# 0215Arthur/Pytorch_News_Recommender

Hardware: AMD Instinct MI355X
Metric: users/sec (train step) NRMS MIND-small hist=50 cand=5 (higher is better)
Workload: dtype f16 (MFMA inputs and saved activations; fp32 accumulate, softmax, loss, master weights and Adam)

## Files before the change

include/nrms_hip.h:

```cpp
#ifndef NRMS_HIP_H
#define NRMS_HIP_H

#include <stddef.h>
#include <stdint.h>

#ifdef __cplusplus
extern "C" {
#endif

#define NRMS_OK            0
#define NRMS_EINVAL       -1
#define NRMS_ELAUNCH      -2
#define NRMS_EWORKSPACE   -3

#define NRMS_PRECISION_FP32   0
#define NRMS_PRECISION_BF16X3 1
#define NRMS_PRECISION_BF16   2
#define NRMS_FP16_KP 320
#define NRMS_FP16_DP 320
#define NRMS_FP16_QP 224
#define NRMS_PRECISION_FP16   3

#define NRMS_FLAG_PAD_ROW_ZERO 1
#define NRMS_FLAG_DEFER_WQKV 2
// ... 46 lines not shown
    float* qkv;
    float* attn;
    float* ctx;
    float* t;
    float* w;
    void*  scratch;
} nrms_encoder_acts;

size_t nrms_encoder_fwd_scratch_bytes(const nrms_encoder_desc* desc);
size_t nrms_encoder_fused_qkv_bytes(const nrms_encoder_desc* desc);
int nrms_encoder_fwd(const nrms_encoder_desc* desc, const nrms_encoder_weights* w,
                     const int64_t* ids, const float* x, const uint8_t* mask ,
                     const nrms_encoder_acts* acts, float* out, void* stream);

size_t nrms_encoder_bwd_workspace_bytes(const nrms_encoder_desc* desc);
int nrms_encoder_bwd(const nrms_encoder_desc* desc, const nrms_encoder_weights* w,
                     const int64_t* ids, const float* x, const uint8_t* mask,
                     const nrms_encoder_acts* acts, const float* dout,
                     const nrms_encoder_grads* grads, float* dx,
                     void* workspace, size_t workspace_bytes, void* stream);
int nrms_encoder_bwd_wqkv(const nrms_encoder_desc* desc, const int64_t* ids, const float* x,
                          const nrms_encoder_acts* acts, const nrms_encoder_grads* grads,
                          void* workspace, size_t workspace_bytes, void* stream);

int nrms_sanitize_ids(const int64_t* src, int64_t* dst, int64_t n, int32_t vocab, int32_t* n_bad, void* stream);
int nrms_sanitize_ids_i32(const int32_t* src, int64_t* dst, int64_t n, int32_t vocab, int32_t* n_bad, void* stream);

int nrms_title_dedup(const int64_t* ids, int64_t n_titles, int32_t seq_len, int32_t* table, int64_t table_size,
                     int32_t* inverse, int32_t* rep_rows, int32_t* n_unique, void* stream);

// ... 118 lines not shown
```

pytorch_news_recommender_amd/_lib.py:

```python
from __future__ import annotations

import ctypes as C
import os

PKG = os.path.dirname(os.path.abspath(__file__))
LIB_PATH = os.environ.get("NRMS_HIP_LIB") or os.path.join(PKG, "libnrms_hip.so")

NRMS_FLAG_PAD_ROW_ZERO = 1
NRMS_FLAG_DEFER_WQKV = 2
NRMS_FLAG_FWD_SCRATCH_KEPT = 4
NRMS_FLAG_FUSED_SEQ64 = 8
NRMS_PRECISION_FP32 = 0
NRMS_PRECISION_BF16X3 = 1
NRMS_PRECISION_BF16 = 2
NRMS_PRECISION_FP16 = 3
NRMS_DROPOUT_FIELDS16 = 0x100
NRMS_FP16_KP, NRMS_FP16_DP, NRMS_FP16_QP = 320, 320, 224
PRECISIONS = {"fp32": 0, "bf16x3": 1, "bf16": 2, "fp16": 3}


class NrmsError(RuntimeError):
    pass


# ... 26 lines not shown


NRMS_SEGPOOL_ROWS_UNIQUE = 1


class NewsFeatures(C.Structure):
    _fields_ = [("n", C.c_int64), ("d_text", C.c_int32), ("d_cat", C.c_int32), ("n_cat", C.c_int32), ("n_sub", C.c_int32),
                ("p_drop", C.c_float), ("seed", C.c_uint64), ("title_vec", C.c_void_p), ("abst_vec", C.c_void_p),
                ("cat_table", C.c_void_p), ("sub_table", C.c_void_p), ("categ", C.c_void_p), ("subcateg", C.c_void_p)]


SIGNATURES = {
    "nrms_encoder_fwd": (C.c_int, [C.POINTER(EncoderDesc), C.POINTER(EncoderWeights), C.c_void_p, C.c_void_p,
                                   C.c_void_p, C.POINTER(EncoderActs), C.c_void_p, C.c_void_p]),
    "nrms_encoder_bwd_workspace_bytes": (C.c_size_t, [C.POINTER(EncoderDesc)]),
    "nrms_encoder_fwd_scratch_bytes": (C.c_size_t, [C.POINTER(EncoderDesc)]),
    "nrms_encoder_fused_qkv_bytes": (C.c_size_t, [C.POINTER(EncoderDesc)]),
    "nrms_encoder_bwd": (C.c_int, [C.POINTER(EncoderDesc), C.POINTER(EncoderWeights), C.c_void_p, C.c_void_p,
                                   C.c_void_p, C.POINTER(EncoderActs), C.c_void_p, C.POINTER(EncoderGrads), C.c_void_p,
                                   C.c_void_p, C.c_size_t, C.c_void_p]),
    "nrms_encoder_bwd_wqkv": (C.c_int, [C.POINTER(EncoderDesc), C.c_void_p, C.c_void_p, C.POINTER(EncoderActs),
                                        C.POINTER(EncoderGrads), C.c_void_p, C.c_size_t, C.c_void_p]),
    "nrms_sanitize_ids": (C.c_int, [C.c_void_p, C.c_void_p, C.c_int64, C.c_int32, C.c_void_p, C.c_void_p]),
    "nrms_sanitize_ids_i32": (C.c_int, [C.c_void_p, C.c_void_p, C.c_int64, C.c_int32, C.c_void_p, C.c_void_p]),
    "nrms_title_dedup": (C.c_int, [C.c_void_p, C.c_int64, C.c_int32, C.c_void_p, C.c_int64, C.c_void_p, C.c_void_p,
                                   C.c_void_p, C.c_void_p]),
    "nrms_click_score_indexed": (C.c_int, [C.c_int32, C.c_int32, C.c_int32, C.c_void_p, C.c_int64, C.c_void_p, C.c_void_p,
                                           C.c_void_p, C.c_void_p, C.c_void_p]),
    "nrms_click_score_fwd": (C.c_int, [C.c_int32, C.c_int32, C.c_int32, C.c_void_p, C.c_void_p, C.c_void_p,
                                       C.c_void_p, C.c_void_p]),
# ... 81 lines not shown
```

pytorch_news_recommender_amd/csrc/capi.hip:

```cpp
#include <stdarg.h>

#include <algorithm>

#include <mutex>
#include <vector>

#include "gemm.h"

namespace nrms {

int launch_attention(bool bwd, int n_seq, int S, int d, int h, const float* qkv, float* ctx, const Dropout& drop,
                     const float* dctx, float* dqkv, const uint8_t* mask, const int64_t* ids, const float* bias_hm,
                     const int* pos, float* padsum, float* dbias, hipStream_t stream, const Dropout* pdrop = nullptr,
                     bool split = false);
size_t attention_padsum_floats();
int launch_addattn_fwd(int n_seq, int S, int d, int q, const float* ctx, const float* w_add, const float* b_add,
                       const float* q_vec, float* T, float* wout, float* out, const uint8_t* mask, int npass,
                       void* wplanes, hipStream_t stream);
int addattn_bwd_rows_waves(int n_seq);
int launch_addattn_bwd_rows(int n_seq, int S, int d, int q, const float* ctx, const float* dout, const float* w,
                            const float* T, float* ds, float* dq_partial, float* dq, const uint8_t* mask,
                            hipStream_t stream);

int launch_attention_wide(bool bwd, int n_seq, int S, int d, int h, const float* qkv, float* ctx, const Dropout& pdrop,
// ... 536 lines not shown
    if (desc->precision == NRMS_PRECISION_FP16) return fwd16_scratch(desc).total;
    return fwd_scratch(desc).total;
}

extern "C" size_t nrms_encoder_fused_qkv_bytes(const nrms_encoder_desc* desc) {
    if (desc == nullptr || !(desc->flags & NRMS_FLAG_FUSED_SEQ64) || validate_desc(desc, "encoder_fused_qkv_bytes")) return 0;
    return user64_qkv_bytes(desc->n_seq, desc->n_heads);
}

extern "C" size_t nrms_encoder_bwd_workspace_bytes(const nrms_encoder_desc* desc) {
    if (validate_desc(desc, "encoder_bwd_workspace_bytes")) return 0;
    if (desc->precision == NRMS_PRECISION_FP16) return bwd16_layout(desc).total;
    return bwd_layout(desc).total;
}

namespace nrms {
struct SideEntry { int device; hipStream_t caller; SideSet* set; };
static std::mutex g_side_mu;
static std::vector<SideEntry> g_side_sets;

SideSet* side_streams_for(hipStream_t caller) {
    if (getenv("NRMS_NO_SIDE_STREAMS") != nullptr) return nullptr;
    int dev = 0;
    if (hipGetDevice(&dev) != hipSuccess) return nullptr;
    std::lock_guard<std::mutex> lk(g_side_mu);
    for (const SideEntry& e : g_side_sets)
        if (e.device == dev && e.caller == caller) return e.set;
    if (g_side_sets.size() >= 32) return nullptr;
    SideSet* ss = new SideSet();
    bool ok = true;
// ... 344 lines not shown
```

pytorch_news_recommender_amd/csrc/fused16_bwd.h:

```cpp
#pragma once
#include "fused16.h"

namespace nrms {

constexpr int B16_RED_QKV = 3 * 10 * 32;
constexpr int B16_RED = B16_RED_QKV + 2 * F16_QP;
constexpr int B16_DQ = 96 * 10;

struct Bwd16Args {
    int n_seq, S, d, h, dk, q;
    int n_groups;
    const _Float16* x16;
    const int* pos;
    const int* n_rows;
    const int64_t* ids;
    const int* order;
    const int* order_cnt;
    int n_cls;
    const _Float16* btiles;
    const float* bqkv32;
    const _Float16* qv16;
    const _Float16* ctx16;
    const _Float16* t16;
    const float* w;
    const _Float16* dout16;
    _Float16* dz16;
    _Float16* dctx16;
    _Float16* dqkv16;
    float* red;
    Dropout drop;
    int v1;
    int dbg;
};

__device__ __forceinline__ f32x16 transpose32(const f32x16& x, const h8 (&idf)[2]) {
    f32x16 z = mfma32h(acc_frag(x, 0), idf[0], zero16());
    return mfma32h(acc_frag(x, 1), idf[1], z);
}

__device__ __forceinline__ float regsum(const f32x16& x) {
    float s0 = 0.f, s1 = 0.f, s2 = 0.f, s3 = 0.f;
#pragma unroll
    for (int g = 0; g < 4; ++g) { s0 += x[4 * g]; s1 += x[4 * g + 1]; s2 += x[4 * g + 2]; s3 += x[4 * g + 3]; }
    return (s0 + s1) + (s2 + s3);
}

__device__ __forceinline__ f32x16 transpose_frags(const h8& x0, const h8& x1, const h8 (&idf)[2]) {
    f32x16 z = mfma32h(x0, idf[0], zero16());
// ... 13 lines not shown
    const _Float16* xtiles;
    int lda, n_slabs;
    float* c;
    int ldc, d;
    const float* sc;
};


size_t bwd16_fused_lds(bool two_blocks);
int launch_bwd16_pool(const Bwd16Args& a, int n_wg, bool two_blocks, hipStream_t stream);
int launch_dx16(const Dx16Args& g, bool out16, hipStream_t stream);
int launch_dout16(long n_seq, int d, int h, int dk, float fixed_scale, float* sc, const float* dout, _Float16* dout16, hipStream_t stream);
int launch_tn16(int geom, const _Float16* A, int lda, int N, const _Float16* B, int ldb, int K, int M, const int* m_dev,
                float* partial, int splits, const int* nmap, const int* kmap, const float* nscale, int ldw, float* dW,
                hipStream_t stream, const char* name, float* dbias = nullptr, const int* blk_list = nullptr, const int* blk_cnt = nullptr,
                int blk_stride = 0);

}
```

pytorch_news_recommender_amd/csrc/fused16_bwd.hip:

```cpp
#include <stdlib.h>

#include "fused16_bwd.h"

namespace nrms {

template <int SB>
__global__ __launch_bounds__(F16_THREADS, SB == 1 ? 8 / F16_WAVES : 1) void fused_bwd16_pool_kernel(Bwd16Args a) {
    extern __shared__ __attribute__((aligned(16))) char smem[];
    float* red = reinterpret_cast<float*>(smem + 3 * F16_SLOT);
    float* stg_t = red + B16_RED;
    float* stg_h = stg_t + F16_WAVES * SB * 2 * F16_QT * 32;
    const int tid = threadIdx.x, lane = tid & 63;
    const int wave = __builtin_amdgcn_readfirstlane(tid >> 6);
    const int l32 = lane & 31, hh = lane >> 5;
    const int S = a.S;
    constexpr int DP = F16_DP, QP = F16_QP;

    for (int i = tid; i < B16_RED; i += F16_THREADS) red[i] = 0.f;

    h8 idf[2], sel[2];
#pragma unroll
    for (int s = 0; s < 2; ++s)
#pragma unroll
        for (int j = 0; j < 8; ++j) {
// ... 84 lines not shown
        for (int b = 0; b < SB; ++b) {
            const float ds = wgt[b] * (dw[b] - aw);
            const _Float16* tsrc = a.t16 + frag_off((long)seq * SB + b, QP / 16, 0, l32, hh);
#pragma unroll
            for (int s = 0; s < 14; ++s) zf[b][s] = *reinterpret_cast<const h8*>(tsrc + 512 * s);
#pragma unroll
            for (int t = 0; t < F16_QT; ++t) {
                f32x16 accz = zero16(), accu = zero16();
#pragma unroll
                for (int s2 = 0; s2 < 2; ++s2) {
                    const int s = 2 * t + s2;
                    const h8 qf = *reinterpret_cast<const h8*>(a.qv16 + 16 * s + 8 * hh);
                    h8 dz, u;
#pragma unroll
                    for (int j = 0; j < 8; ++j) {
                        const float tv = (float)zf[b][s][j];
                        dz[j] = (_Float16)(ds * (float)qf[j] * (1.0f - tv * tv));
                        u[j] = (_Float16)(ds * tv);
                    }
                    zf[b][s] = dz;
                    if (valid && !F16_DBG(a.dbg, 4)) *reinterpret_cast<h8*>(a.dz16 + frag_off((long)seq * SB + b, QP / 16, s, l32, hh)) = dz;
                    accz = mfma32h(dz, sel[s2], accz);
                    accu = mfma32h(u, sel[s2], accu);
                }
                float cz = valid ? regsum(accz) : 0.f, cu = valid ? regsum(accu) : 0.f;
                cz += __shfl_xor(cz, 32, 64);
                cu += __shfl_xor(cu, 32, 64);
                if (hh == 0) {
                    float* row = stg_t + ((wave * SB + b) * 2 * F16_QT + 2 * t) * 32 + l32;
                    row[0] = cz;
                    row[32] = cu;
                }
            }
            zf[b][14] = h8{0, 0, 0, 0, 0, 0, 0, 0};
            zf[b][15] = h8{0, 0, 0, 0, 0, 0, 0, 0};
        }
        ring.store(0);
        ring.load(1);
        ring.store(1);
        const bool any_closed = __syncthreads_or((!live && valid) ? 1 : 0) != 0;
        for (int i = tid; i < 2 * F16_QT * 32; i += F16_THREADS) {
            float sum = 0.f;
#pragma unroll
            for (int w = 0; w < F16_WAVES; ++w)
#pragma unroll
                for (int b = 0; b < SB; ++b) sum += stg_t[((w * SB + b) * 2 * F16_QT) * 32 + i];
            const int r = i >> 5, c = i & 31;
            red[B16_RED_QKV + (r & 1) * QP + 32 * (r >> 1) + c] += sum;
        }

        int n = 0;
#pragma unroll 1
        for (int head = 0; head < a.h; ++head) {
            ring.load(n + 2);
            const h8 d0 = *reinterpret_cast<const h8*>(a.dout16 + (long)seq * DP + head * 32 + 8 * hh);
            const h8 d1 = *reinterpret_cast<const h8*>(a.dout16 + (long)seq * DP + head * 32 + 16 + 8 * hh);
            float closed = 0.f;
#pragma unroll
            for (int b = 0; b < SB; ++b) {
                f32x16 dct = zero16();
                if (!F16_DBG(a.dbg, 8)) tile_mma<true>(dct, ring, n, zf[b]);
#pragma unroll
                for (int r = 0; r < 8; ++r) {
                    dct[r] += wgt[b] * (float)d0[r];
                    dct[8 + r] += wgt[b] * (float)d1[r];
                }
                if (a.drop.thresh != 0u) {
#pragma unroll
                    for (int c = 0; c < 2; ++c) {
                        const uint64_t e0 = (uint64_t)(tok0 + 32 * b + l32) * (uint64_t)DP + (uint64_t)(head * 32 + 16 * c + 8 * hh);
                        float sc[8];
// ... 551 lines not shown
    static constexpr int STAGE = A_BYTES + B_BYTES;
    static constexpr int A_IT = (T16_MC * AW / 8 + T16_THREADS - 1) / T16_THREADS;
    static constexpr int B_IT = (T16_MC * BW / 8 + T16_THREADS - 1) / T16_THREADS;
};
typedef Tn16Geom<4, 5, 2, 5> Tn16Qkv;
typedef Tn16Geom<2, 7, 4, 5> Tn16Add;

struct Tn16Args {
    int M;
    const int* m_dev;
    const _Float16* A; int lda, N;
    const _Float16* B; int ldb, K;
    float* partial;
    int splits, n_blk, k_blk;
    const int* blk_list; const int* blk_cnt; int blk_stride;
};

typedef short s16x4 __attribute__((ext_vector_type(4)));
typedef short s16x8 __attribute__((ext_vector_type(8)));

__device__ __forceinline__ h8 tr16_frag(const char* plane, int pitch_b, int col0, int lane) {
    const int l16 = lane & 15, kq = lane >> 4;
    const int q = l16 >> 2, p = l16 & 3;
    const char* a0 = plane + (4 * kq + q) * pitch_b + (col0 + 4 * p) * 2;
    const s16x4 lo4 = __builtin_amdgcn_ds_read_tr16_b64_v4i16((s16x4 __attribute__((address_space(3)))*)(a0));
    const s16x4 hi4 = __builtin_amdgcn_ds_read_tr16_b64_v4i16((s16x4 __attribute__((address_space(3)))*)(a0 + 16 * pitch_b));
    s16x8 r;
#pragma unroll
    for (int i = 0; i < 4; ++i) { r[i] = lo4[i]; r[4 + i] = hi4[i]; }
    return __builtin_bit_cast(h8, r);
}

template <bool FL, int WN, int NTN, int WK, int NTK>
__global__ __launch_bounds__(T16_THREADS, 2) void gemm16_tn_kernel(Tn16Args a) {
    typedef Tn16Geom<WN, NTN, WK, NTK> G;
    constexpr int T16_AW = G::AW, T16_BW = G::BW, T16_PA = G::PA, T16_PB = G::PB, T16_A_BYTES = G::A_BYTES;
    constexpr int T16_STAGE = G::STAGE, T16_A_IT = G::A_IT, T16_B_IT = G::B_IT, T16_NTN = NTN, T16_NTK = NTK;
    extern __shared__ __attribute__((aligned(16))) char smem[];
    const int tid = threadIdx.x, lane = tid & 63;
    const int wave = __builtin_amdgcn_readfirstlane(tid >> 6);
    const int wn = wave / WK, wk = wave % WK;
    const int out_blocks = a.n_blk * a.k_blk;
    const int per_xcd = gridDim.x >> 3;
    const int idx = (gridDim.x & 7) == 0 ? (blockIdx.x & 7) * per_xcd + (blockIdx.x >> 3) : blockIdx.x;
    const int blk = idx % out_blocks, split = idx / out_blocks;
    const int bn = blk % a.n_blk, bk = blk / a.n_blk;
    const int ncol0 = bn * T16_AW, kcol0 = bk * T16_BW;
    const int n_list0 = (FL && a.blk_list != nullptr) ? a.blk_cnt[0] : 0;
    const int M = (FL && a.blk_list != nullptr) ? 32 * (n_list0 + a.blk_cnt[2]) : (a.m_dev != nullptr ? *a.m_dev : a.M);
    const int rps = (((M + a.splits - 1) / a.splits) + T16_MC - 1) / T16_MC * T16_MC;
    const int m_begin = split * rps, m_end = min(M, m_begin + rps);

    struct Regs { h8 a[T16_A_IT], b[T16_B_IT]; };
    auto slot_rc = [&](int sl, int width, int& r, int& c) {
        if (FL) { r = (sl >> 1) & 31; c = (sl >> 6) * 16 + (sl & 1) * 8; if (c >= width) r = T16_MC; }
        else { r = sl / (width / 8); c = (sl % (width / 8)) * 8; }
    };
    auto load_stage = [&](Regs& R, int m0) {
        long blk = min(m0, max(m_end - 1, 0)) >> 5;
        if (FL && a.blk_list != nullptr && M > 0) blk = blk < n_list0 ? a.blk_list[blk] : a.blk_list[2 * (long)a.blk_stride + blk - n_list0];
#pragma unroll
        for (int i = 0; i < T16_A_IT; ++i) {
            int r, c;
            slot_rc(tid + T16_THREADS * i, T16_AW, r, c);
            r = min(r, T16_MC - 1);
            const int cc = min(ncol0 + c, a.N - 8);
            if (FL) R.a[i] = *reinterpret_cast<const h8*>(a.A + (blk * (a.lda >> 4) + (cc >> 4)) * 512 + r * 16 + (cc & 8));
            else R.a[i] = *reinterpret_cast<const h8*>(a.A + (long)min(m0 + r, max(m_end - 1, 0)) * a.lda + cc);
        }
#pragma unroll
        for (int i = 0; i < T16_B_IT; ++i) {
            int r, c;
            slot_rc(tid + T16_THREADS * i, T16_BW, r, c);
            r = min(r, T16_MC - 1);
            const int cc = min(kcol0 + c, a.K - 8);
            if (FL) R.b[i] = *reinterpret_cast<const h8*>(a.B + (blk * (a.ldb >> 4) + (cc >> 4)) * 512 + r * 16 + (cc & 8));
            else R.b[i] = *reinterpret_cast<const h8*>(a.B + (long)min(m0 + r, max(m_end - 1, 0)) * a.ldb + cc);
        }
    };
    const h8 z8 = {0, 0, 0, 0, 0, 0, 0, 0};
    auto store_stage = [&](const Regs& R, int m0, char* st) {
#pragma unroll
        for (int i = 0; i < T16_A_IT; ++i) {
            int r, c;
            slot_rc(tid + T16_THREADS * i, T16_AW, r, c);
            if (r < T16_MC) {
                const bool ok = m0 + r < m_end && ncol0 + c < a.N;
                *reinterpret_cast<h8*>(st + (r * T16_PA + c) * 2) = ok ? R.a[i] : z8;
            }
        }
#pragma unroll
        for (int i = 0; i < T16_B_IT; ++i) {
            int r, c;
            slot_rc(tid + T16_THREADS * i, T16_BW, r, c);
            if (r < T16_MC) {
                const bool ok = m0 + r < m_end && kcol0 + c < a.K;
                *reinterpret_cast<h8*>(st + T16_A_BYTES + (r * T16_PB + c) * 2) = ok ? R.b[i] : z8;
            }
        }
    };
    f32x4 acc[T16_NTN][T16_NTK];
#pragma unroll
    for (int i = 0; i < T16_NTN; ++i)
// ... 125 lines not shown

static size_t up256(size_t x) { return (x + 255) / 256 * 256; }


Fused16BwdLayout fused16_bwd_layout(long M, int n_seq) {
    Fused16BwdLayout L;
    const long Mp = (long)n_seq * (M > (long)n_seq * 32 ? 64 : 32);
    size_t off = 0;
    auto take = [&](size_t bytes) { size_t o = off; off = up256(off + bytes); return o; };
    L.n_wg = 512;
    L.btiles = take((size_t)40 * 32 * F16_KP * 2);
    L.xtiles = take((size_t)DX_SLABS * DX_B_BYTES);
    L.qv16 = take((size_t)F16_QP * 2);
    L.bqkv32 = take((size_t)30 * 32 * 4);
    L.dout16 = take((size_t)n_seq * F16_DP * 2);
    L.dz16 = take((size_t)Mp * F16_QP * 2);
    L.dctx16 = take((size_t)Mp * F16_DP * 2);
    L.dqkv16 = take((size_t)(M + 32) * B16_DQ * 2);
    L.red = take((size_t)2 * L.n_wg * B16_RED * 4);
    L.maps = take((size_t)(B16_DQ * 2 + F16_KP + F16_QP * 2 + F16_DP) * 4);
    L.scale = take(256);
    L.tn_splits_qkv = 40;
    L.tn_splits_add = 192;
    if (const char* e = getenv("NRMS_TN_SPLITS_QKV")) L.tn_splits_qkv = atoi(e);
    if (const char* e = getenv("NRMS_TN_SPLITS_ADD")) L.tn_splits_add = atoi(e);
    const size_t p1 = (size_t)L.tn_splits_qkv * B16_DQ * F16_KP * 4, p2 = (size_t)L.tn_splits_add * F16_QP * F16_DP * 4;
    L.partial = take(up256(p1) + p2);
    L.total = off;
    return L;
}

int launch_tn16(int geom, const _Float16* A, int lda, int N, const _Float16* B, int ldb, int K, int M, const int* m_dev,
                float* partial, int splits, const int* nmap, const int* kmap, const float* nscale, int ldw, float* dW,
                hipStream_t stream, const char* name, float* dbias, const int* blk_list, const int* blk_cnt, int blk_stride) {
    Tn16Args t{};
    t.M = M; t.m_dev = m_dev; t.A = A; t.lda = lda; t.N = N; t.B = B; t.ldb = ldb; t.K = K; t.partial = partial;
    t.blk_list = geom != 0 ? blk_list : nullptr; t.blk_cnt = blk_cnt; t.blk_stride = blk_stride;
    typedef void (*Kern)(Tn16Args);
    const Kern fn = geom == 1 ? (Kern)gemm16_tn_kernel<true, 2, 7, 4, 5> : geom == 2 ? (Kern)gemm16_tn_kernel<true, 4, 5, 2, 5>
                                                                                     : (Kern)gemm16_tn_kernel<false, 4, 5, 2, 5>;
    const int aw = geom == 1 ? Tn16Add::AW : Tn16Qkv::AW, bw = geom == 1 ? Tn16Add::BW : Tn16Qkv::BW;
    t.splits = splits; t.n_blk = cdiv(N, aw); t.k_blk = cdiv(K, bw);
    const size_t lds = 2 * (size_t)(geom == 1 ? Tn16Add::STAGE : Tn16Qkv::STAGE);
    const hipError_t e = hipFuncSetAttribute((const void*)fn, hipFuncAttributeMaxDynamicSharedMemorySize, (int)lds);
    if (e != hipSuccess) { set_error("%s: hipFuncSetAttribute: %s", name, hipGetErrorString(e)); return NRMS_ELAUNCH; }
    {
        TimingScope ts(name, stream);
        hipLaunchKernelGGL(fn, dim3(splits * t.n_blk * t.k_blk), dim3(T16_THREADS), lds, stream, t);
    }
    int rc = check_launch(name);
    if (rc) return rc;
    TimingScope ts("tn_reduce", stream);
    hipLaunchKernelGGL(tn16_reduce_kernel, dim3(cdiv((long)N * K, 256)), dim3(256), 0, stream, partial, splits, N, K, nmap, kmap,
                       nscale, ldw, dW, dbias);
    return check_launch("tn16_reduce");
// ... 38 lines not shown
    return check_launch("dout16");
}

int launch_fused_bwd16(const Fused16Bwd& f, hipStream_t stream) {
    if (f.n_seq <= 0) return NRMS_OK;
    const long M = (long)f.n_seq * f.S;
    const Fused16BwdLayout L = fused16_bwd_layout(M, f.n_seq);
    char* base = (char*)f.workspace;
    const int dk = f.d / f.h;
    const float qscale = 1.0f / sqrtf((float)dk);
    _Float16* btiles = (_Float16*)(base + L.btiles);
    _Float16* xtiles = (_Float16*)(base + L.xtiles);
    _Float16* qv16 = (_Float16*)(base + L.qv16);
    float* bqkv32 = (float*)(base + L.bqkv32);
    _Float16* dout16 = (_Float16*)(base + L.dout16);
    _Float16* dz16 = (_Float16*)(base + L.dz16);
    _Float16* dctx16 = (_Float16*)(base + L.dctx16);
    _Float16* dqkv16 = (_Float16*)(base + L.dqkv16);
    float* red = (float*)(base + L.red);
    int* nmap_qkv = (int*)(base + L.maps);
    float* nscale_qkv = (float*)(nmap_qkv + B16_DQ);
    int* kmap_x = (int*)(nscale_qkv + B16_DQ);
    int* nmap_add = kmap_x + F16_KP;
    float* nscale_add = (float*)(nmap_add + F16_QP);
    int* kmap_ctx = (int*)(nscale_add + F16_QP);
    float* sc = (float*)(base + L.scale);
    if (f.sc_out != nullptr) *f.sc_out = sc;
    float* partial_qkv = (float*)(base + L.partial);
    float* partial_add = (float*)(base + L.partial + up256((size_t)L.tn_splits_qkv * B16_DQ * F16_KP * 4));
    { const int jr = fused_bwd16_join(stream); if (jr) return jr; }
    SideSet* ss = side_streams_for(stream);
// ... 9 lines not shown
        hipLaunchKernelGGL(prep16b_kernel, dim3(2048), dim3(256), 0, stream, p);
        int rc0 = launch_dout16((long)f.n_seq, f.d, f.h, dk, f.loss_scale, sc, f.dout, dout16, stream);
        if (rc0) return rc0;
        hipLaunchKernelGGL(maps16_kernel, dim3(cdiv(B16_DQ, 256)), dim3(256), 0, stream, f.d, f.h, dk, f.q, sc, qscale,
                           nmap_qkv, nscale_qkv, kmap_x, nmap_add, nscale_add, kmap_ctx);
        int rc = check_launch("prep16b");
        if (rc) return rc;
    }
    Bwd16Args a{};
    a.n_seq = f.n_seq; a.S = f.S; a.d = f.d; a.h = f.h; a.dk = dk; a.q = f.q;
    a.n_groups = cdiv(f.n_seq, F16_WAVES) + (f.order != nullptr ? 2 : 0);
    a.n_cls = f.order != nullptr ? 3 : 2;
    a.x16 = (const _Float16*)f.x16; a.pos = f.pos; a.n_rows = f.n_rows_dev; a.ids = f.ids; a.order = f.order; a.order_cnt = f.order_cnt;
    a.btiles = btiles; a.bqkv32 = bqkv32; a.qv16 = qv16;
    a.ctx16 = (const _Float16*)f.ctx16; a.t16 = (const _Float16*)f.t16; a.w = f.w; a.dout16 = dout16;
    a.dz16 = dz16; a.dctx16 = dctx16; a.dqkv16 = dqkv16; a.red = red; a.drop = f.drop;
    a.dbg = 0;
#ifdef NRMS_F16_EXPERIMENTS
    { const char* e = getenv("NRMS_F16_DBG"); a.dbg = e ? atoi(e) : 0; }
#endif
    const int n_wg = a.n_groups < L.n_wg ? a.n_groups : L.n_wg;
    {
        const bool two = f.S > 32;
        const size_t lds = bwd16_fused_lds(two);
        const void* fa = two ? (const void*)fused_bwd16_attn_kernel<2> : (const void*)fused_bwd16_attn_kernel<1>;
        const hipError_t e = hipFuncSetAttribute(fa, hipFuncAttributeMaxDynamicSharedMemorySize, (int)lds);
        if (e != hipSuccess) { set_error("fused_bwd16: hipFuncSetAttribute: %s", hipGetErrorString(e)); return NRMS_ELAUNCH; }
        {
            const int rcp = launch_bwd16_pool(a, n_wg, two, stream);
            if (rcp) return rcp;
        }
        if (side) {
            int rc = side_order(ss, 0, stream, s_add, "fused_bwd16");
            if (rc) return rc;
            rc = launch_tn16(1, dz16, F16_QP, F16_QP, (const _Float16*)f.ctx16, F16_DP, F16_DP, Mp, nullptr, partial_add,
                             L.tn_splits_add, nmap_add, kmap_ctx, nscale_add, f.d, f.dw_add, s_add, "dwadd_bwd");
            if (rc) return rc;
            if (hipEventRecord(ss->ev[2], s_add) != hipSuccess) { set_error("fused_bwd16: hipEventRecord failed"); return NRMS_ELAUNCH; }
        }
        Bwd16Args b = a;
        b.red = red + (long)n_wg * B16_RED;
        {
            TimingScope ts(two ? "fused64_bwd16_attn" : "fused_bwd16_attn", stream);
            if (two) hipLaunchKernelGGL(fused_bwd16_attn_kernel<2>, dim3(n_wg), dim3(F16_THREADS), lds, stream, b);
            else hipLaunchKernelGGL(fused_bwd16_attn_kernel<1>, dim3(n_wg), dim3(F16_THREADS), lds, stream, b);
        }
        int rc = check_launch("fused_bwd16");
        if (rc) return rc;
    }
    {
        TimingScope ts("red16", stream);
        hipLaunchKernelGGL(red16_kernel, dim3(cdiv(B16_RED, 32)), dim3(1024), 0, stream, red, 2 * n_wg, f.h, dk, f.d, f.q, sc,
                           qscale, f.db_qkv, f.db_add, f.dq_vec);
        int rc = check_launch("red16");
        if (rc) return rc;
    }
    int rc = NRMS_OK;
    if (!side) {
        rc = launch_tn16(1, dz16, F16_QP, F16_QP, (const _Float16*)f.ctx16, F16_DP, F16_DP, Mp, nullptr, partial_add,
                         L.tn_splits_add, nmap_add, kmap_ctx, nscale_add, f.d, f.dw_add, stream, "dwadd_bwd");
        if (rc) return rc;
    }
    if (side) {
        rc = side_order(ss, 1, stream, s_qkv, "fused_bwd16");
        if (rc) return rc;
    }
    rc = launch_tn16(0, dqkv16, B16_DQ, B16_DQ, (const _Float16*)f.x16, F16_KP, F16_KP, (int)M, f.n_rows_dev, partial_qkv,
                     L.tn_splits_qkv, nmap_qkv, kmap_x, nscale_qkv, f.d, f.dw_qkv, s_qkv, "dwqkv_bwd");
    if (rc) return rc;
    if (side && hipEventRecord(ss->ev[3], s_qkv) != hipSuccess) { set_error("fused_bwd16: hipEventRecord failed"); return NRMS_ELAUNCH; }
    {
        Dx16Args g{};
        g.M = (int)M; g.m_dev = f.n_rows_dev; g.a16 = dqkv16; g.xtiles = xtiles; g.c = f.dx; g.ldc = f.d; g.d = f.d;
        g.sc = sc; g.lda = B16_DQ; g.n_slabs = DX_SLABS;
        rc = launch_dx16(g, f.dx_fp16, stream);
// ... 25 lines not shown
```

pytorch_news_recommender_amd/csrc/fused16_v1_bwd.hip:

```cpp
#include <stdlib.h>

#include "fused16_bwd.h"
#include "fused16_v1.h"

namespace nrms {

constexpr int V1_RED = 36 * 32;
constexpr int V1_HMAX = 6;

struct Bwd16V1Args {
    int n_seq, S;
    V1Geom g;
    const _Float16* x16;
    const int* pos;
    const int* n_rows;
    const int64_t* ids;
    const int* order;
    const int* order_cnt;
    const _Float16* btiles;
    const _Float16* dctx16;
    _Float16* scratch;
    _Float16* dqkv16;
    float* red;
};
// ... 415 lines not shown
    if (c < g.d)
        for (int o = og; o < g.d; o += 32) s += w_o[(long)o * g.d + c] * ebuf[(o / g.dkv) * 32 + o % g.dkv];
    part[og][cl] = s;
    __syncthreads();
    if (og != 0 || c >= g.d) return;
    s = 0.f;
#pragma unroll
    for (int r = 0; r < 32; ++r) s += part[r][cl];
    db_qkv[2 * g.d + c] += s;
}

static size_t up256(size_t x) { return (x + 255) / 256 * 256; }

struct Fused16V1BwdLayout {
    int n_wg, splits_qkv, splits_add, splits_o;
    size_t btiles, xtiles, qv16, dout16, dz16, dctx16, scratch, dqkv16, red_pool, red_attn, ebuf, maps, scale, p_qkv, p_add, p_o, total;
};

static Fused16V1BwdLayout v1_bwd_layout(long M, int n_seq, int h) {
    Fused16V1BwdLayout L;
    const long Mp = (long)n_seq * 32;
    size_t off = 0;
    auto take = [&](size_t bytes) { size_t o = off; off = up256(off + bytes); return o; };
    L.n_wg = 512;
    L.btiles = take((size_t)(10 + 8 * h) * 32 * F16_KP * 2);
    L.xtiles = take((size_t)3 * h * DX_B_BYTES);
    L.qv16 = take((size_t)F16_QP * 2);
    L.dout16 = take((size_t)n_seq * F16_DP * 2);
    L.dz16 = take((size_t)Mp * F16_QP * 2);
    L.dctx16 = take((size_t)Mp * F16_DP * 2);
    L.scratch = take((size_t)L.n_wg * F16_WAVES * 4 * h * 1024);
    L.dqkv16 = take((size_t)(M + 32) * 192 * h * 2);
    L.red_pool = take((size_t)L.n_wg * B16_RED * 4);
    L.red_attn = take((size_t)L.n_wg * V1_RED * 4);
    L.ebuf = take((size_t)10 * 32 * 4);
    L.maps = take((size_t)(192 * V1_HMAX * 2 + F16_KP + F16_QP * 2 + F16_DP * 3) * 4);
    L.scale = take(256);
    const int nb = cdiv(192 * h, 320) * 2;
    L.splits_qkv = 240 / nb;
    L.splits_add = 192;
    L.splits_o = 64;
    if (const char* e = getenv("NRMS_TN_SPLITS_QKV")) L.splits_qkv = atoi(e);
    if (const char* e = getenv("NRMS_TN_SPLITS_ADD")) L.splits_add = atoi(e);
    if (const char* e = getenv("NRMS_TN_SPLITS_O")) L.splits_o = atoi(e);
// ... 9 lines not shown
int launch_fused_bwd16v1(const Fused16Bwd& f, hipStream_t stream) {
    if (f.n_seq <= 0) return NRMS_OK;
    if (f.order == nullptr || f.pos == nullptr || f.ids == nullptr || f.n_rows_dev == nullptr || f.S > 32 || f.h > V1_HMAX ||
        f.w_o == nullptr || f.attn16 == nullptr || f.dw_o == nullptr || f.db_o == nullptr) {
        set_error("fused_bwd16v1: needs the padding-skipping path (pos, ids, order lists), seq_len <= 32, w_o / attn16 / dw_o / db_o");
        return NRMS_EINVAL;
    }
    const long M = (long)f.n_seq * f.S;
    const V1Geom g = v1_geom(f.d, f.h);
    const Fused16V1BwdLayout L = v1_bwd_layout(M, f.n_seq, f.h);
    char* base = (char*)f.workspace;
    _Float16* btiles = (_Float16*)(base + L.btiles);
    _Float16* xtiles = (_Float16*)(base + L.xtiles);
    _Float16* qv16 = (_Float16*)(base + L.qv16);
    _Float16* dout16 = (_Float16*)(base + L.dout16);
    _Float16* dz16 = (_Float16*)(base + L.dz16);
    _Float16* dctx16 = (_Float16*)(base + L.dctx16);
    _Float16* dqkv16 = (_Float16*)(base + L.dqkv16);
    float* red_pool = (float*)(base + L.red_pool);
    float* red_attn = (float*)(base + L.red_attn);
    float* ebuf = (float*)(base + L.ebuf);
    Maps16V1 mp;
    mp.nmap_qkv = (int*)(base + L.maps);
    mp.nscale_qkv = (float*)(mp.nmap_qkv + 192 * V1_HMAX);
    mp.kmap_x = (int*)(mp.nscale_qkv + 192 * V1_HMAX);
    mp.nmap_add = mp.kmap_x + F16_KP;
    mp.nscale_add = (float*)(mp.nmap_add + F16_QP);
    mp.kmap_ctx = (int*)(mp.nscale_add + F16_QP);
    mp.nscale_o = (float*)(mp.kmap_ctx + F16_DP);
    mp.kmap_attn = (int*)(mp.nscale_o + F16_DP);
    float* sc = (float*)(base + L.scale);
// ... 14 lines not shown
        rc = launch_dout16((long)f.n_seq, f.d, g.hv, g.dkv, f.loss_scale, sc, f.dout, dout16, stream);
        if (rc) return rc;
        hipLaunchKernelGGL(maps16v1_kernel, dim3(cdiv(192 * V1_HMAX, 256)), dim3(256), 0, stream, g, f.q, sc, mp);
        rc = check_launch("prep16bv1");
        if (rc) return rc;
    }
    const int n_groups = cdiv(f.n_seq, F16_WAVES) + 2;
    const int n_wg = n_groups < L.n_wg ? n_groups : L.n_wg;
    {
        Bwd16Args a{};
        a.n_seq = f.n_seq; a.S = f.S; a.d = f.d; a.h = g.hv; a.dk = g.dkv; a.q = f.q;
        a.n_groups = n_groups; a.n_cls = 3;
        a.x16 = (const _Float16*)f.x16; a.pos = f.pos; a.n_rows = f.n_rows_dev; a.ids = f.ids; a.order = f.order; a.order_cnt = f.order_cnt;
        a.btiles = btiles; a.bqkv32 = nullptr; a.qv16 = qv16;
        a.ctx16 = (const _Float16*)f.ctx16; a.t16 = (const _Float16*)f.t16; a.w = f.w; a.dout16 = dout16;
        a.dz16 = dz16; a.dctx16 = dctx16; a.dqkv16 = nullptr; a.red = red_pool; a.drop = f.drop;
        a.v1 = 1; a.dbg = 0;
        rc = launch_bwd16_pool(a, n_wg, false, stream);
        if (rc) return rc;
        TimingScope ts("red16", stream);
        hipLaunchKernelGGL(red16v1_kernel, dim3(cdiv(B16_RED, 32)), dim3(1024), 0, stream, 0, red_pool, n_wg, g, f.q, sc,
                           f.db_qkv, f.db_add, f.dq_vec, ebuf);
        rc = check_launch("red16v1");
        if (rc) return rc;
    }
    if (side) { rc = side_order(ss, 0, stream, s_add, "fused_bwd16v1"); if (rc) return rc; }
    rc = launch_tn16(1, dz16, F16_QP, F16_QP, (const _Float16*)f.ctx16, F16_DP, F16_DP, Mp, nullptr, (float*)(base + L.p_add),
                     L.splits_add, mp.nmap_add, mp.kmap_ctx, mp.nscale_add, f.d, f.dw_add, s_add, "dwadd_bwd");
    if (rc) return rc;
    rc = launch_tn16(2, dctx16, F16_DP, F16_DP, (const _Float16*)f.attn16, F16_DP, F16_DP, Mp, nullptr, (float*)(base + L.p_o),
                     L.splits_o, mp.kmap_ctx, mp.kmap_attn, mp.nscale_o, f.d, f.dw_o, s_add, "dwo_bwd", f.db_o, f.order, f.order_cnt, f.n_seq);
    if (rc) return rc;
    {
        TimingScope ts("closed16", s_add);
        hipLaunchKernelGGL(closed16v1_wo_kernel, dim3(cdiv(f.d * f.d, 256)), dim3(256), 0, s_add, g, f.b_qkv, ebuf, f.dw_o, f.db_o);
        rc = check_launch("closed16v1_wo");
        if (rc) return rc;
    }
    if (side && hipEventRecord(ss->ev[2], s_add) != hipSuccess) { set_error("fused_bwd16v1: hipEventRecord failed"); return NRMS_ELAUNCH; }
    {
        Bwd16V1Args b{};
        b.n_seq = f.n_seq; b.S = f.S; b.g = g;
        b.x16 = (const _Float16*)f.x16; b.pos = f.pos; b.n_rows = f.n_rows_dev; b.ids = f.ids; b.order = f.order; b.order_cnt = f.order_cnt;
// ... 42 lines not shown
```

pytorch_news_recommender_amd/csrc/gemm.h:

```cpp
#pragma once
#include "common.h"

namespace nrms {

constexpr int NT_BM = 128;
constexpr int NT_BK = 16;
constexpr int NT_STAGE_A = NT_BM * NT_BK;

enum { A_PLAIN = 0, A_DZ = 2 };
enum { E_STORE = 0, E_DCTX = 1 };

struct NTArgs {
    int M, N, K;
    int rows_per_tile;
    const float* A; int lda;
    const float* ds;
    const float* qv;
    const float* T;
    const float* W;
    const float* bias;
    float* C; int ldc;
    const float* wrow;
    const float* dout;
    int S;
// ... 259 lines not shown
    void* ctx16;
    void* t16;
    float* w;
    float* out;
    Dropout drop;
};
int launch_fused_fwd16(const Fused16Fwd& f, hipStream_t stream);
bool fused16v1_supported(int S, int d, int h, int q, const char** why);
size_t fused16v1_planes_bytes(int d, int h, int q);
int launch_prep16v1(int d, int h, int q, const float* w_qkv, const float* b_qkv, const float* w_o, const float* b_o,
                    const float* w_add, const float* b_add, const float* q_vec, void* planes, hipStream_t stream);
int launch_fused_fwd16v1(const Fused16Fwd& f, int h, void* attn16, hipStream_t stream);
size_t title_order_cnt_ints(int n_seq);
int launch_title_order(int n_seq, int S, const int64_t* ids, int* order, int* cnt, hipStream_t stream, int n_classes = 2);

struct Fused16BwdLayout { int n_wg, tn_splits_qkv, tn_splits_add; size_t btiles, xtiles, qv16, bqkv32, dout16, dz16, dctx16, dqkv16, red, maps, scale, partial, total; };
Fused16BwdLayout fused16_bwd_layout(long M, int n_seq);
struct Fused16Bwd {
    int n_seq, S, d, h, q;
    void* workspace;
    const float* w_qkv; const float* b_qkv; const float* w_add; const float* q_vec;
    const void* x16;
    const int* pos;
    const int* n_rows_dev;
    const int64_t* ids;
    const int* order; const int* order_cnt;
    const void* ctx16; const void* t16; const float* w;
    const float* dout;
    float loss_scale;
    Dropout drop;
    float* dw_qkv; float* db_qkv; float* dw_add; float* db_add; float* dq_vec;
// ... 47 lines not shown
```

Before: 170,000.

## Recompute additive-attention dZ inside dW_add GEMM from saved t16 and per-row ds

The backward pool kernel no longer writes the full fp16 dZ matrix (Mp x QP). It now stores one fp32 ds scalar per row, and the dW_add TN GEMM rebuilds dZ = ds*q*(1-t^2) from the saved forward tanh activations t16 while staging A tiles. This cuts a large write and reread of global memory at the cost of extra ALU work and per-row ds loads in the GEMM staging path. A small load reordering in the head loop is also included. A new C API exposes the ds and scale offsets in the workspace.

```diff
diff --git a/include/nrms_hip.h b/include/nrms_hip.h
--- a/include/nrms_hip.h
+++ b/include/nrms_hip.h
@@ -84,6 +84,7 @@
                      const nrms_encoder_acts* acts, float* out, void* stream);
 
 size_t nrms_encoder_bwd_workspace_bytes(const nrms_encoder_desc* desc);
+size_t nrms_encoder_bwd16_plane_offset(const nrms_encoder_desc* desc, int32_t which);
 int nrms_encoder_bwd(const nrms_encoder_desc* desc, const nrms_encoder_weights* w,
                      const int64_t* ids, const float* x, const uint8_t* mask,
                      const nrms_encoder_acts* acts, const float* dout,
diff --git a/pytorch_news_recommender_amd/_lib.py b/pytorch_news_recommender_amd/_lib.py
--- a/pytorch_news_recommender_amd/_lib.py
+++ b/pytorch_news_recommender_amd/_lib.py
@@ -64,6 +64,7 @@
     "nrms_encoder_fwd": (C.c_int, [C.POINTER(EncoderDesc), C.POINTER(EncoderWeights), C.c_void_p, C.c_void_p,
                                    C.c_void_p, C.POINTER(EncoderActs), C.c_void_p, C.c_void_p]),
     "nrms_encoder_bwd_workspace_bytes": (C.c_size_t, [C.POINTER(EncoderDesc)]),
+    "nrms_encoder_bwd16_plane_offset": (C.c_size_t, [C.POINTER(EncoderDesc), C.c_int32]),
     "nrms_encoder_fwd_scratch_bytes": (C.c_size_t, [C.POINTER(EncoderDesc)]),
     "nrms_encoder_fused_qkv_bytes": (C.c_size_t, [C.POINTER(EncoderDesc)]),
     "nrms_encoder_bwd": (C.c_int, [C.POINTER(EncoderDesc), C.POINTER(EncoderWeights), C.c_void_p, C.c_void_p,
diff --git a/pytorch_news_recommender_amd/csrc/capi.hip b/pytorch_news_recommender_amd/csrc/capi.hip
--- a/pytorch_news_recommender_amd/csrc/capi.hip
+++ b/pytorch_news_recommender_amd/csrc/capi.hip
@@ -574,6 +574,13 @@
     return bwd_layout(desc).total;
 }
 
+extern "C" size_t nrms_encoder_bwd16_plane_offset(const nrms_encoder_desc* desc, int32_t which) {
+    if (validate_desc(desc, "encoder_bwd16_plane_offset")) return (size_t)-1;
+    if (desc->precision != NRMS_PRECISION_FP16 || desc->use_output_proj || (which != 0 && which != 1)) return (size_t)-1;
+    const Fused16BwdLayout F = fused16_bwd_layout((long)desc->n_seq * desc->seq_len, desc->n_seq);
+    return bwd16_layout(desc).fused + (which == 0 ? F.ds : F.scale);
+}
+
 namespace nrms {
 struct SideEntry { int device; hipStream_t caller; SideSet* set; };
 static std::mutex g_side_mu;
diff --git a/pytorch_news_recommender_amd/csrc/fused16_bwd.h b/pytorch_news_recommender_amd/csrc/fused16_bwd.h
--- a/pytorch_news_recommender_amd/csrc/fused16_bwd.h
+++ b/pytorch_news_recommender_amd/csrc/fused16_bwd.h
@@ -24,7 +24,7 @@
     const _Float16* t16;
     const float* w;
     const _Float16* dout16;
-    _Float16* dz16;
+    float* ds;
     _Float16* dctx16;
     _Float16* dqkv16;
     float* red;
@@ -32,6 +32,11 @@
     int v1;
     int dbg;
 };
+
+__device__ __forceinline__ _Float16 dz16_elem(float ds, _Float16 q, _Float16 t) {
+    const float tv = (float)t;
+    return (_Float16)(ds * (float)q * __builtin_fmaf(-tv, tv, 1.0f));
+}
 
 __device__ __forceinline__ f32x16 transpose32(const f32x16& x, const h8 (&idf)[2]) {
     f32x16 z = mfma32h(acc_frag(x, 0), idf[0], zero16());
@@ -75,6 +80,7 @@
 int launch_tn16(int geom, const _Float16* A, int lda, int N, const _Float16* B, int ldb, int K, int M, const int* m_dev,
                 float* partial, int splits, const int* nmap, const int* kmap, const float* nscale, int ldw, float* dW,
                 hipStream_t stream, const char* name, float* dbias = nullptr, const int* blk_list = nullptr, const int* blk_cnt = nullptr,
-                int blk_stride = 0);
+                int blk_stride = 0,
+                const float* ds = nullptr, const _Float16* qv = nullptr);
 
 }
diff --git a/pytorch_news_recommender_amd/csrc/fused16_bwd.hip b/pytorch_news_recommender_amd/csrc/fused16_bwd.hip
--- a/pytorch_news_recommender_amd/csrc/fused16_bwd.hip
+++ b/pytorch_news_recommender_amd/csrc/fused16_bwd.hip
@@ -122,12 +122,10 @@
                     h8 dz, u;
 #pragma unroll
                     for (int j = 0; j < 8; ++j) {
-                        const float tv = (float)zf[b][s][j];
-                        dz[j] = (_Float16)(ds * (float)qf[j] * (1.0f - tv * tv));
-                        u[j] = (_Float16)(ds * tv);
+                        dz[j] = dz16_elem(ds, qf[j], zf[b][s][j]);
+                        u[j] = (_Float16)(ds * (float)zf[b][s][j]);
                     }
                     zf[b][s] = dz;
-                    if (valid && !F16_DBG(a.dbg, 4)) *reinterpret_cast<h8*>(a.dz16 + frag_off((long)seq * SB + b, QP / 16, s, l32, hh)) = dz;
                     accz = mfma32h(dz, sel[s2], accz);
                     accu = mfma32h(u, sel[s2], accu);
                 }
@@ -142,6 +140,7 @@
             }
             zf[b][14] = h8{0, 0, 0, 0, 0, 0, 0, 0};
             zf[b][15] = h8{0, 0, 0, 0, 0, 0, 0, 0};
+            if (valid && hh == 0 && !F16_DBG(a.dbg, 4)) a.ds[((long)seq * SB + b) * 32 + l32] = ds;
         }
         ring.store(0);
         ring.load(1);
@@ -160,9 +159,9 @@
         int n = 0;
 #pragma unroll 1
         for (int head = 0; head < a.h; ++head) {
-            ring.load(n + 2);
             const h8 d0 = *reinterpret_cast<const h8*>(a.dout16 + (long)seq * DP + head * 32 + 8 * hh);
             const h8 d1 = *reinterpret_cast<const h8*>(a.dout16 + (long)seq * DP + head * 32 + 16 + 8 * hh);
+            ring.load(n + 2);
             float closed = 0.f;
 #pragma unroll
             for (int b = 0; b < SB; ++b) {
@@ -744,6 +743,8 @@
     float* partial;
     int splits, n_blk, k_blk;
     const int* blk_list; const int* blk_cnt; int blk_stride;
+    const float* ds;
+    const _Float16* qv;
 };
 
 typedef short s16x4 __attribute__((ext_vector_type(4)));
@@ -761,8 +762,9 @@
     return __builtin_bit_cast(h8, r);
 }
 
-template <bool FL, int WN, int NTN, int WK, int NTK>
+template <bool FL, bool DZ, int WN, int NTN, int WK, int NTK>
 __global__ __launch_bounds__(T16_THREADS, 2) void gemm16_tn_kernel(Tn16Args a) {
+    static_assert(FL || !DZ, "dZ rows are addressed in fragment order");
     typedef Tn16Geom<WN, NTN, WK, NTK> G;
     constexpr int T16_AW = G::AW, T16_BW = G::BW, T16_PA = G::PA, T16_PB = G::PB, T16_A_BYTES = G::A_BYTES;
     constexpr int T16_STAGE = G::STAGE, T16_A_IT = G::A_IT, T16_B_IT = G::B_IT, T16_NTN = NTN, T16_NTK = NTK;
@@ -781,7 +783,7 @@
     const int rps = (((M + a.splits - 1) / a.splits) + T16_MC - 1) / T16_MC * T16_MC;
     const int m_begin = split * rps, m_end = min(M, m_begin + rps);
 
-    struct Regs { h8 a[T16_A_IT], b[T16_B_IT]; };
+    struct Regs { h8 a[T16_A_IT], b[T16_B_IT]; float ds[DZ ? T16_A_IT : 1]; };
     auto slot_rc = [&](int sl, int width, int& r, int& c) {
         if (FL) { r = (sl >> 1) & 31; c = (sl >> 6) * 16 + (sl & 1) * 8; if (c >= width) r = T16_MC; }
         else { r = sl / (width / 8); c = (sl % (width / 8)) * 8; }
@@ -797,6 +799,7 @@
             const int cc = min(ncol0 + c, a.N - 8);
             if (FL) R.a[i] = *reinterpret_cast<const h8*>(a.A + (blk * (a.lda >> 4) + (cc >> 4)) * 512 + r * 16 + (cc & 8));
             else R.a[i] = *reinterpret_cast<const h8*>(a.A + (long)min(m0 + r, max(m_end - 1, 0)) * a.lda + cc);
+            if (DZ) R.ds[i] = a.ds[blk * 32 + r];
         }
 #pragma unroll
         for (int i = 0; i < T16_B_IT; ++i) {
@@ -809,6 +812,15 @@
         }
     };
     const h8 z8 = {0, 0, 0, 0, 0, 0, 0, 0};
+    h8 qv[DZ ? T16_A_IT : 1];
+    if (DZ) {
+#pragma unroll
+        for (int i = 0; i < T16_A_IT; ++i) {
+            int r, c;
+            slot_rc(tid + T16_THREADS * i, T16_AW, r, c);
+            qv[i] = *reinterpret_cast<const h8*>(a.qv + min(ncol0 + c, a.N - 8));
+        }
+    }
     auto store_stage = [&](const Regs& R, int m0, char* st) {
 #pragma unroll
         for (int i = 0; i < T16_A_IT; ++i) {
@@ -816,7 +828,12 @@
             slot_rc(tid + T16_THREADS * i, T16_AW, r, c);
             if (r < T16_MC) {
                 const bool ok = m0 + r < m_end && ncol0 + c < a.N;
-                *reinterpret_cast<h8*>(st + (r * T16_PA + c) * 2) = ok ? R.a[i] : z8;
+                h8 v = R.a[i];
+                if (DZ) {
+#pragma unroll
+                    for (int j = 0; j < 8; ++j) v[j] = dz16_elem(R.ds[i], qv[i][j], R.a[i][j]);
+                }
+                *reinterpret_cast<h8*>(st + (r * T16_PA + c) * 2) = ok ? v : z8;
             }
         }
 #pragma unroll
@@ -972,7 +989,7 @@
     L.qv16 = take((size_t)F16_QP * 2);
     L.bqkv32 = take((size_t)30 * 32 * 4);
     L.dout16 = take((size_t)n_seq * F16_DP * 2);
-    L.dz16 = take((size_t)Mp * F16_QP * 2);
+    L.ds = take((size_t)Mp * 4);
     L.dctx16 = take((size_t)Mp * F16_DP * 2);
     L.dqkv16 = take((size_t)(M + 32) * B16_DQ * 2);
     L.red = take((size_t)2 * L.n_wg * B16_RED * 4);
@@ -990,13 +1007,17 @@
 
 int launch_tn16(int geom, const _Float16* A, int lda, int N, const _Float16* B, int ldb, int K, int M, const int* m_dev,
                 float* partial, int splits, const int* nmap, const int* kmap, const float* nscale, int ldw, float* dW,
-                hipStream_t stream, const char* name, float* dbias, const int* blk_list, const int* blk_cnt, int blk_stride) {
+                hipStream_t stream, const char* name, float* dbias, const int* blk_list, const int* blk_cnt, int blk_stride,
+                const float* ds, const _Float16* qv) {
+    if (geom == 1 && (ds == nullptr || qv == nullptr)) { set_error("%s: the d(W_add) product needs ds and qv16", name); return NRMS_EINVAL; }
     Tn16Args t{};
     t.M = M; t.m_dev = m_dev; t.A = A; t.lda = lda; t.N = N; t.B = B; t.ldb = ldb; t.K = K; t.partial = partial;
     t.blk_list = geom != 0 ? blk_list : nullptr; t.blk_cnt = blk_cnt; t.blk_stride = blk_stride;
+    t.ds = ds; t.qv = qv;
     typedef void (*Kern)(Tn16Args);
-    const Kern fn = geom == 1 ? (Kern)gemm16_tn_kernel<true, 2, 7, 4, 5> : geom == 2 ? (Kern)gemm16_tn_kernel<true, 4, 5, 2, 5>
-                                                                                     : (Kern)gemm16_tn_kernel<false, 4, 5, 2, 5>;
+    const Kern fn = geom == 1 ? (Kern)gemm16_tn_kernel<true, true, 2, 7, 4, 5>
+                  : geom == 2 ? (Kern)gemm16_tn_kernel<true, false, 4, 5, 2, 5>
+                              : (Kern)gemm16_tn_kernel<false, false, 4, 5, 2, 5>;
     const int aw = geom == 1 ? Tn16Add::AW : Tn16Qkv::AW, bw = geom == 1 ? Tn16Add::BW : Tn16Qkv::BW;
     t.splits = splits; t.n_blk = cdiv(N, aw); t.k_blk = cdiv(K, bw);
     const size_t lds = 2 * (size_t)(geom == 1 ? Tn16Add::STAGE : Tn16Qkv::STAGE);
@@ -1065,7 +1086,7 @@
     _Float16* qv16 = (_Float16*)(base + L.qv16);
     float* bqkv32 = (float*)(base + L.bqkv32);
     _Float16* dout16 = (_Float16*)(base + L.dout16);
-    _Float16* dz16 = (_Float16*)(base + L.dz16);
+    float* ds = (float*)(base + L.ds);
     _Float16* dctx16 = (_Float16*)(base + L.dctx16);
     _Float16* dqkv16 = (_Float16*)(base + L.dqkv16);
     float* red = (float*)(base + L.red);
@@ -1105,7 +1126,7 @@
     a.x16 = (const _Float16*)f.x16; a.pos = f.pos; a.n_rows = f.n_rows_dev; a.ids = f.ids; a.order = f.order; a.order_cnt = f.order_cnt;
     a.btiles = btiles; a.bqkv32 = bqkv32; a.qv16 = qv16;
     a.ctx16 = (const _Float16*)f.ctx16; a.t16 = (const _Float16*)f.t16; a.w = f.w; a.dout16 = dout16;
-    a.dz16 = dz16; a.dctx16 = dctx16; a.dqkv16 = dqkv16; a.red = red; a.drop = f.drop;
+    a.ds = ds; a.dctx16 = dctx16; a.dqkv16 = dqkv16; a.red = red; a.drop = f.drop;
     a.dbg = 0;
 #ifdef NRMS_F16_EXPERIMENTS
     { const char* e = getenv("NRMS_F16_DBG"); a.dbg = e ? atoi(e) : 0; }
@@ -1124,8 +1145,9 @@
         if (side) {
             int rc = side_order(ss, 0, stream, s_add, "fused_bwd16");
             if (rc) return rc;
-            rc = launch_tn16(1, dz16, F16_QP, F16_QP, (const _Float16*)f.ctx16, F16_DP, F16_DP, Mp, nullptr, partial_add,
-                             L.tn_splits_add, nmap_add, kmap_ctx, nscale_add, f.d, f.dw_add, s_add, "dwadd_bwd");
+            rc = launch_tn16(1, (const _Float16*)f.t16, F16_QP, F16_QP, (const _Float16*)f.ctx16, F16_DP, F16_DP, Mp, nullptr, partial_add,
+                             L.tn_splits_add, nmap_add, kmap_ctx, nscale_add, f.d, f.dw_add, s_add, "dwadd_bwd", nullptr, nullptr,
+                             nullptr, 0, ds, qv16);
             if (rc) return rc;
             if (hipEventRecord(ss->ev[2], s_add) != hipSuccess) { set_error("fused_bwd16: hipEventRecord failed"); return NRMS_ELAUNCH; }
         }
@@ -1148,8 +1170,9 @@
     }
     int rc = NRMS_OK;
     if (!side) {
-        rc = launch_tn16(1, dz16, F16_QP, F16_QP, (const _Float16*)f.ctx16, F16_DP, F16_DP, Mp, nullptr, partial_add,
-                         L.tn_splits_add, nmap_add, kmap_ctx, nscale_add, f.d, f.dw_add, stream, "dwadd_bwd");
+        rc = launch_tn16(1, (const _Float16*)f.t16, F16_QP, F16_QP, (const _Float16*)f.ctx16, F16_DP, F16_DP, Mp, nullptr, partial_add,
+                         L.tn_splits_add, nmap_add, kmap_ctx, nscale_add, f.d, f.dw_add, stream, "dwadd_bwd", nullptr, nullptr,
+                         nullptr, 0, ds, qv16);
         if (rc) return rc;
     }
     if (side) {
diff --git a/pytorch_news_recommender_amd/csrc/fused16_v1_bwd.hip b/pytorch_news_recommender_amd/csrc/fused16_v1_bwd.hip
--- a/pytorch_news_recommender_amd/csrc/fused16_v1_bwd.hip
+++ b/pytorch_news_recommender_amd/csrc/fused16_v1_bwd.hip
@@ -453,7 +453,7 @@
 
 struct Fused16V1BwdLayout {
     int n_wg, splits_qkv, splits_add, splits_o;
-    size_t btiles, xtiles, qv16, dout16, dz16, dctx16, scratch, dqkv16, red_pool, red_attn, ebuf, maps, scale, p_qkv, p_add, p_o, total;
+    size_t btiles, xtiles, qv16, dout16, ds, dctx16, scratch, dqkv16, red_pool, red_attn, ebuf, maps, scale, p_qkv, p_add, p_o, total;
 };
 
 static Fused16V1BwdLayout v1_bwd_layout(long M, int n_seq, int h) {
@@ -466,7 +466,7 @@
     L.xtiles = take((size_t)3 * h * DX_B_BYTES);
     L.qv16 = take((size_t)F16_QP * 2);
     L.dout16 = take((size_t)n_seq * F16_DP * 2);
-    L.dz16 = take((size_t)Mp * F16_QP * 2);
+    L.ds = take((size_t)Mp * 4);
     L.dctx16 = take((size_t)Mp * F16_DP * 2);
     L.scratch = take((size_t)L.n_wg * F16_WAVES * 4 * h * 1024);
     L.dqkv16 = take((size_t)(M + 32) * 192 * h * 2);
@@ -506,7 +506,7 @@
     _Float16* xtiles = (_Float16*)(base + L.xtiles);
     _Float16* qv16 = (_Float16*)(base + L.qv16);
     _Float16* dout16 = (_Float16*)(base + L.dout16);
-    _Float16* dz16 = (_Float16*)(base + L.dz16);
+    float* ds = (float*)(base + L.ds);
     _Float16* dctx16 = (_Float16*)(base + L.dctx16);
     _Float16* dqkv16 = (_Float16*)(base + L.dqkv16);
     float* red_pool = (float*)(base + L.red_pool);
@@ -551,7 +551,7 @@
         a.x16 = (const _Float16*)f.x16; a.pos = f.pos; a.n_rows = f.n_rows_dev; a.ids = f.ids; a.order = f.order; a.order_cnt = f.order_cnt;
         a.btiles = btiles; a.bqkv32 = nullptr; a.qv16 = qv16;
         a.ctx16 = (const _Float16*)f.ctx16; a.t16 = (const _Float16*)f.t16; a.w = f.w; a.dout16 = dout16;
-        a.dz16 = dz16; a.dctx16 = dctx16; a.dqkv16 = nullptr; a.red = red_pool; a.drop = f.drop;
+        a.ds = ds; a.dctx16 = dctx16; a.dqkv16 = nullptr; a.red = red_pool; a.drop = f.drop;
         a.v1 = 1; a.dbg = 0;
         rc = launch_bwd16_pool(a, n_wg, false, stream);
         if (rc) return rc;
@@ -562,8 +562,9 @@
         if (rc) return rc;
     }
     if (side) { rc = side_order(ss, 0, stream, s_add, "fused_bwd16v1"); if (rc) return rc; }
-    rc = launch_tn16(1, dz16, F16_QP, F16_QP, (const _Float16*)f.ctx16, F16_DP, F16_DP, Mp, nullptr, (float*)(base + L.p_add),
-                     L.splits_add, mp.nmap_add, mp.kmap_ctx, mp.nscale_add, f.d, f.dw_add, s_add, "dwadd_bwd");
+    rc = launch_tn16(1, (const _Float16*)f.t16, F16_QP, F16_QP, (const _Float16*)f.ctx16, F16_DP, F16_DP, Mp, nullptr,
+                     (float*)(base + L.p_add), L.splits_add, mp.nmap_add, mp.kmap_ctx, mp.nscale_add, f.d, f.dw_add, s_add, "dwadd_bwd",
+                     nullptr, nullptr, nullptr, 0, ds, qv16);
     if (rc) return rc;
     rc = launch_tn16(2, dctx16, F16_DP, F16_DP, (const _Float16*)f.attn16, F16_DP, F16_DP, Mp, nullptr, (float*)(base + L.p_o),
                      L.splits_o, mp.kmap_ctx, mp.kmap_attn, mp.nscale_o, f.d, f.dw_o, s_add, "dwo_bwd", f.db_o, f.order, f.order_cnt, f.n_seq);
diff --git a/pytorch_news_recommender_amd/csrc/gemm.h b/pytorch_news_recommender_amd/csrc/gemm.h
--- a/pytorch_news_recommender_amd/csrc/gemm.h
+++ b/pytorch_news_recommender_amd/csrc/gemm.h
@@ -297,7 +297,7 @@
 size_t title_order_cnt_ints(int n_seq);
 int launch_title_order(int n_seq, int S, const int64_t* ids, int* order, int* cnt, hipStream_t stream, int n_classes = 2);
 
-struct Fused16BwdLayout { int n_wg, tn_splits_qkv, tn_splits_add; size_t btiles, xtiles, qv16, bqkv32, dout16, dz16, dctx16, dqkv16, red, maps, scale, partial, total; };
+struct Fused16BwdLayout { int n_wg, tn_splits_qkv, tn_splits_add; size_t btiles, xtiles, qv16, bqkv32, dout16, ds, dctx16, dqkv16, red, maps, scale, partial, total; };
 Fused16BwdLayout fused16_bwd_layout(long M, int n_seq);
 struct Fused16Bwd {
     int n_seq, S, d, h, q;
```

Result: no change. 170,700, median of 6 (+0.5%).
